# ubc-vision/StableKeypoints

Hardware: AMD Instinct MI355X
Metric: images/sec for token-optimization step (SD1.5, 512^2, K=10 kpts) (higher is better)
Workload: dtype f32 (fp32 MFMA / VALU throughout; flash attention of the >= 1024-key self-attention layers: 3xbf16 operand split, fp32 accumulate, error <= the fp32 kernel's)

## Files before the change

### stablekeypoints_amd/csrc/skp_flash_attn_s.hip

```cpp
#include "skp_attn_tiles.h"
#include <stdlib.h>

typedef __bf16 bf16x8 __attribute__((ext_vector_type(8)));

namespace {

template <int D>
struct FAS {
    static constexpr int G = (D + 15) / 16;
    static constexpr int KT = 64, NKT = 4;
    static constexpr int MAT_B = NKT * G * 2 * 1024;
    static constexpr int CHUNKS = MAT_B / 1024;
    static constexpr bool ONES = (D % 16) != 0;
};

__device__ __forceinline__ unsigned fas_cvt_pk(float lo, float hi) {
    unsigned r;
    asm("v_cvt_pk_bf16_f32 %0, %1, %2" : "=v"(r) : "v"(lo), "v"(hi));
    return r;
}
__device__ __forceinline__ void fas_split4(const f32x4 a, f32x4& mh, f32x4& hl) {
    unsigned h[2], m[2], l[2];
#pragma unroll
    for (int p = 0; p < 2; ++p) {
        const float x = a[2 * p], y = a[2 * p + 1];
        h[p] = fas_cvt_pk(x, y);
        const float rx = x - __builtin_bit_cast(float, h[p] << 16), ry = y - __builtin_bit_cast(float, h[p] & 0xffff0000u);
        m[p] = fas_cvt_pk(rx, ry);
        const float sx = rx - __builtin_bit_cast(float, m[p] << 16), sy = ry - __builtin_bit_cast(float, m[p] & 0xffff0000u);
        l[p] = fas_cvt_pk(sx, sy);
    }
    mh = f32x4{__builtin_bit_cast(float, m[0]), __builtin_bit_cast(float, h[0]), __builtin_bit_cast(float, m[1]), __builtin_bit_cast(float, h[1])};
    hl = f32x4{__builtin_bit_cast(float, h[0]), __builtin_bit_cast(float, l[0]), __builtin_bit_cast(float, h[1]), __builtin_bit_cast(float, l[1])};
}
__device__ __forceinline__ f32x4 fas_mfma(const f32x4& a, const f32x4& b, const f32x4& c) {
    return __builtin_amdgcn_mfma_f32_16x16x32_bf16(__builtin_bit_cast(bf16x8, a), __builtin_bit_cast(bf16x8, b), c, 0, 0, 0);
}

template <int D>
__global__ __launch_bounds__(256) void skp_fas_split_kernel(const float* __restrict__ k, const float* __restrict__ v, f32x4* __restrict__ Kt,
                                                           f32x4* __restrict__ Vt, int H, int Nk, int ntiles) {
    using F = FAS<D>;
    const int cell = blockIdx.x * 256 + threadIdx.x;
    const int lane = cell & 63, rest = cell >> 6;
    const int g = rest % F::G, kt = (rest / F::G) % F::NKT, tile = rest / (F::G * F::NKT);
    if (tile >= ntiles) return;
    const int h = blockIdx.y, bk = blockIdx.z, C = H * D;
    const int i16 = lane & 15, kq = lane >> 4;
    const float* kb = k + (size_t)bk * Nk * C + h * D;
    const float* vb = v + (size_t)bk * Nk * C + h * D;
    f32x4 a = {0.f, 0.f, 0.f, 0.f}, b = {0.f, 0.f, 0.f, 0.f};
    {
        const int t = tile * F::KT + 16 * kt + i16, c = 16 * g + 4 * kq;
        if (t < Nk && c < D) a = *(const f32x4*)(kb + (size_t)t * C + c);
    }
    {
        const int c = 16 * g + i16, t0 = tile * F::KT + 16 * kt + 4 * kq;
#pragma unroll
        for (int e = 0; e < 4; ++e)
            if (t0 + e < Nk) b[e] = c < D ? vb[(size_t)(t0 + e) * C + c] : (F::ONES && c == D ? 1.0f : 0.f);
    }
    f32x4 mh, hl;
    const size_t base = (((size_t)(bk * H + h) * ntiles + tile) * (F::MAT_B / 16)) + ((kt * F::G + g) * 2) * 64 + lane;
    fas_split4(a, mh, hl);
    Kt[base] = mh; Kt[base + 64] = hl;
    fas_split4(b, mh, hl);
    Vt[base] = mh; Vt[base + 64] = hl;
}

template <int D, int NQT>
__global__ __launch_bounds__(512, 2) void skp_fas_fwd_kernel(const float* __restrict__ q, const float* __restrict__ Kt, const float* __restrict__ Vt,
                                                            float* __restrict__ out, float* __restrict__ lse, int H, int N, int Nk,
                                                            int ntiles, int kvb, float scale) {
    using F = FAS<D>;
    extern __shared__ __attribute__((aligned(16))) unsigned char smem[];
    const int tid = threadIdx.x, lane = tid & 63, wave = __builtin_amdgcn_readfirstlane(tid >> 6);
    const int i16 = lane & 15, g = lane >> 4;
    const int b = blockIdx.z, h = blockIdx.y, C = H * D;
    const int nbase = blockIdx.x * (128 * NQT) + wave * (16 * NQT);
    const float sl2 = scale * SKP_LOG2E;
    const size_t img = (size_t)((kvb ? b : 0) * H + h) * ntiles * F::MAT_B;
    const i32x4 krs = skp_make_rsrc((const char*)Kt + img, (unsigned)((size_t)ntiles * F::MAT_B));
    const i32x4 vrs = skp_make_rsrc((const char*)Vt + img, (unsigned)((size_t)ntiles * F::MAT_B));

    f32x4 qmh[NQT][F::G], qhl[NQT][F::G];
    int nrow[NQT];
#pragma unroll
    for (int nt = 0; nt < NQT; ++nt) {
        const int n = nbase + 16 * nt + i16;
        nrow[nt] = n;
        const float* qrow = q + ((size_t)b * N + (n < N ? n : N - 1)) * C + h * D;
#pragma unroll
        for (int gg = 0; gg < F::G; ++gg) {
            const int c = 16 * gg + 4 * g;
            const f32x4 x = c < D ? *(const f32x4*)(qrow + c) * sl2 : f32x4{0.f, 0.f, 0.f, 0.f};
            fas_split4(x, qmh[nt][gg], qhl[nt][gg]);
        }
    }
    f32x4 o[F::G][NQT];
#pragma unroll
    for (int ct = 0; ct < F::G; ++ct)
#pragma unroll
        for (int nt = 0; nt < NQT; ++nt) o[ct][nt] = f32x4{0.f, 0.f, 0.f, 0.f};
    float mrun[NQT], lpart[NQT];
#pragma unroll
    for (int nt = 0; nt < NQT; ++nt) { mrun[nt] = -INFINITY; lpart[nt] = 0.f; }
    constexpr int LCT = D / 16, LG = (D % 16) / 4, LR = D % 4;

    auto stage = [&](int tile, int buf) {
        unsigned char* dst = smem + buf * 2 * F::MAT_B;
#pragma unroll
        for (int j = 0; j < (F::CHUNKS + 7) / 8; ++j) {
            const int p = j * 8 + wave;
            if (p < F::CHUNKS) {
                skp_buf_load_lds(krs, (skp_lds_ptr)(dst + p * 1024), 16, lane * 16, tile * F::MAT_B + p * 1024, 0, 0);
                skp_buf_load_lds(vrs, (skp_lds_ptr)(dst + F::MAT_B + p * 1024), 16, lane * 16, tile * F::MAT_B + p * 1024, 0, 0);
            }
        }
    };
    stage(0, 0);
    for (int tile = 0; tile < ntiles; ++tile) {
        const int cur = tile & 1;
        asm volatile("s_waitcnt vmcnt(0)" ::: "memory");
        __syncthreads();
        if (tile + 1 < ntiles) stage(tile + 1, cur ^ 1);
        const unsigned char* Ks = smem + cur * 2 * F::MAT_B + lane * 16;
        const unsigned char* Vs = Ks + F::MAT_B;
        const int kt0 = tile * F::KT;

        f32x4 s[F::NKT][NQT];
#pragma unroll
        for (int kt = 0; kt < F::NKT; ++kt) {
#pragma unroll
            for (int nt = 0; nt < NQT; ++nt) s[kt][nt] = f32x4{0.f, 0.f, 0.f, 0.f};
#pragma unroll
            for (int gg = 0; gg < F::G; ++gg) {
                const f32x4 kmh = *(const f32x4*)(Ks + ((kt * F::G + gg) * 2) * 1024);
                const f32x4 khl = *(const f32x4*)(Ks + ((kt * F::G + gg) * 2 + 1) * 1024);
#pragma unroll
                for (int nt = 0; nt < NQT; ++nt) s[kt][nt] = fas_mfma(kmh, qhl[nt][gg], s[kt][nt]);
#pragma unroll
                for (int nt = 0; nt < NQT; ++nt) s[kt][nt] = fas_mfma(khl, qmh[nt][gg], s[kt][nt]);
#pragma unroll
                for (int nt = 0; nt < NQT; ++nt) s[kt][nt] = fas_mfma(kmh, qmh[nt][gg], s[kt][nt]);
            }
        }
        if (kt0 + F::KT > Nk) {
            const int left = Nk - kt0;
#pragma unroll
            for (int kt = 0; kt < F::NKT; ++kt)
#pragma unroll
                for (int r = 0; r < 4; ++r)
                    if (16 * kt + 4 * g + r >= left) {
#pragma unroll
                        for (int nt = 0; nt < NQT; ++nt) s[kt][nt][r] = -INFINITY;
                    }
        }
#pragma unroll
        for (int nt = 0; nt < NQT; ++nt) {
            float tm = fmaxf(fmaxf(s[0][nt][0], s[0][nt][1]), fmaxf(s[0][nt][2], s[0][nt][3]));
#pragma unroll
            for (int kt = 1; kt < F::NKT; ++kt) tm = fmaxf(tm, fmaxf(fmaxf(s[kt][nt][0], s[kt][nt][1]), fmaxf(s[kt][nt][2], s[kt][nt][3])));
            tm = fmaxf(tm, __shfl_xor(tm, 16, 64));
            tm = fmaxf(tm, __shfl_xor(tm, 32, 64));
            const float mn = fmaxf(mrun[nt], tm);
            const float alpha = __builtin_amdgcn_exp2f(mrun[nt] - mn);
            mrun[nt] = mn;
            float rs = 0.f;
#pragma unroll
            for (int kt = 0; kt < F::NKT; ++kt)
#pragma unroll
                for (int r = 0; r < 4; ++r) {
                    s[kt][nt][r] = __builtin_amdgcn_exp2f(s[kt][nt][r] - mn);
                    if (!F::ONES) rs += s[kt][nt][r];
                }
            if (!F::ONES) lpart[nt] = lpart[nt] * alpha + rs;
#pragma unroll
            for (int ct = 0; ct < F::G; ++ct) o[ct][nt] *= alpha;
        }
#pragma unroll
        for (int kt = 0; kt < F::NKT; ++kt) {
            f32x4 pmh[NQT], phl[NQT];
#pragma unroll
            for (int nt = 0; nt < NQT; ++nt) fas_split4(s[kt][nt], pmh[nt], phl[nt]);
#pragma unroll
            for (int ct = 0; ct < F::G; ++ct) {
                const f32x4 vmh = *(const f32x4*)(Vs + ((kt * F::G + ct) * 2) * 1024);
                const f32x4 vhl = *(const f32x4*)(Vs + ((kt * F::G + ct) * 2 + 1) * 1024);
#pragma unroll
                for (int nt = 0; nt < NQT; ++nt) o[ct][nt] = fas_mfma(vmh, phl[nt], o[ct][nt]);
#pragma unroll
                for (int nt = 0; nt < NQT; ++nt) o[ct][nt] = fas_mfma(vhl, pmh[nt], o[ct][nt]);
#pragma unroll
                for (int nt = 0; nt < NQT; ++nt) o[ct][nt] = fas_mfma(vmh, pmh[nt], o[ct][nt]);
            }
        }
    }
#pragma unroll
    for (int nt = 0; nt < NQT; ++nt) {
        float l;
        if (F::ONES) l = __shfl(o[LCT][nt][LR], 16 * LG + i16, 64);
        else { l = lpart[nt]; l += __shfl_xor(l, 16, 64); l += __shfl_xor(l, 32, 64); }
        const float inv = 1.0f / l;
        const int n = nrow[nt];
        if (n < N) {
            float* orow = out + ((size_t)b * N + n) * C + h * D;
#pragma unroll
            for (int ct = 0; ct < F::G; ++ct) {
                const int c0 = 16 * ct + 4 * g;
                if (c0 < D) *(f32x4*)(orow + c0) = o[ct][nt] * inv;
            }
            if (g == 0) lse[((size_t)b * H + h) * N + n] = (mrun[nt] + __builtin_amdgcn_logf(l)) * SKP_LN2;
        }
    }
}

template <int D, int NB>
__global__ __launch_bounds__(256) void skp_fas_images_kernel(const float* __restrict__ x, f32x4* __restrict__ Xr, f32x4* __restrict__ Xt, int H,
                                                            int Nr, int ntiles, float mult) {
    using F = FAS<D>;
    constexpr int MAT16 = NB * F::G * 2 * 64;
    const int cell = blockIdx.x * 256 + threadIdx.x;
    const int lane = cell & 63, rest = cell >> 6;
    const int g = rest % F::G, nb = (rest / F::G) % NB, tile = rest / (F::G * NB);
    if (tile >= ntiles) return;
    const int h = blockIdx.y, b = blockIdx.z, C = H * D;
    const int i16 = lane & 15, kq = lane >> 4;
    const float* xb = x + (size_t)b * Nr * C + h * D;
    f32x4 a = {0.f, 0.f, 0.f, 0.f}, t4 = {0.f, 0.f, 0.f, 0.f};
    {
        const int r = tile * 16 * NB + 16 * nb + i16, c = 16 * g + 4 * kq;
        if (r < Nr && c < D) a = *(const f32x4*)(xb + (size_t)r * C + c) * mult;
    }
    {
        const int c = 16 * g + i16, r0 = tile * 16 * NB + 16 * nb + 4 * kq;
#pragma unroll
        for (int e = 0; e < 4; ++e)
            if (r0 + e < Nr && c < D) t4[e] = xb[(size_t)(r0 + e) * C + c] * mult;
    }
    f32x4 mh, hl;
    const size_t base = ((size_t)(b * H + h) * ntiles + tile) * MAT16 + ((nb * F::G + g) * 2) * 64 + lane;
    fas_split4(a, mh, hl);
    Xr[base] = mh; Xr[base + 64] = hl;
    fas_split4(t4, mh, hl);
    Xt[base] = mh; Xt[base + 64] = hl;
}

template <int D>
__global__ __launch_bounds__(512, 2) void skp_fas_bwd_dq_kernel(const float* __restrict__ q, const float* __restrict__ o, const float* __restrict__ dout,
                                                               const float* __restrict__ lse, const float* __restrict__ Kr,
                                                               const float* __restrict__ Vr, const float* __restrict__ Kt,
                                                               float* __restrict__ dq, float* __restrict__ Dn, int H, int N, int Nk,
                                                               int ntiles, float scale, int ldg) {
    using F = FAS<D>;
    constexpr int NQT = 2;
    extern __shared__ __attribute__((aligned(16))) unsigned char smem[];
    const int tid = threadIdx.x, lane = tid & 63, wave = __builtin_amdgcn_readfirstlane(tid >> 6);
    const int i16 = lane & 15, g = lane >> 4;
    const int b = blockIdx.z, h = blockIdx.y, C = H * D;
    const int nbase = blockIdx.x * 256 + wave * (16 * NQT);
    const float sl2 = scale * SKP_LOG2E;
    const size_t img = (size_t)(b * H + h) * ntiles * F::MAT_B;
    const i32x4 krs = skp_make_rsrc((const char*)Kr + img, (unsigned)((size_t)ntiles * F::MAT_B));
    const i32x4 vrs = skp_make_rsrc((const char*)Vr + img, (unsigned)((size_t)ntiles * F::MAT_B));
    const i32x4 trs = skp_make_rsrc((const char*)Kt + img, (unsigned)((size_t)ntiles * F::MAT_B));

    f32x4 qmh[NQT][F::G], qhl[NQT][F::G], gmh[NQT][F::G], ghl[NQT][F::G];
    float lse2[NQT], dsum[NQT];
    int nrow[NQT];
#pragma unroll
    for (int nt = 0; nt < NQT; ++nt) {
        const int n = nbase + 16 * nt + i16;
        nrow[nt] = n;
        const size_t ro = ((size_t)b * N + (n < N ? n : N - 1)) * C + h * D;
        float dpart = 0.f;
#pragma unroll
        for (int gg = 0; gg < F::G; ++gg) {
            const int c = 16 * gg + 4 * g;
            f32x4 x = {0.f, 0.f, 0.f, 0.f}, gv = {0.f, 0.f, 0.f, 0.f}, ov = {0.f, 0.f, 0.f, 0.f};
            if (c < D) { x = *(const f32x4*)(q + ro + c) * sl2; gv = *(const f32x4*)(dout + ro + c); ov = *(const f32x4*)(o + ro + c); }
            fas_split4(x, qmh[nt][gg], qhl[nt][gg]);
            fas_split4(gv, gmh[nt][gg], ghl[nt][gg]);
            dpart += gv[0] * ov[0] + gv[1] * ov[1] + gv[2] * ov[2] + gv[3] * ov[3];
        }
        dpart += __shfl_xor(dpart, 16, 64);
        dpart += __shfl_xor(dpart, 32, 64);
        dsum[nt] = dpart;
        lse2[nt] = lse[((size_t)b * H + h) * N + (n < N ? n : N - 1)] * SKP_LOG2E;
        if (g == 0 && n < N) Dn[((size_t)b * H + h) * N + n] = dpart;
    }
    f32x4 acc[F::G][NQT];
#pragma unroll
    for (int ct = 0; ct < F::G; ++ct)
#pragma unroll
        for (int nt = 0; nt < NQT; ++nt) acc[ct][nt] = f32x4{0.f, 0.f, 0.f, 0.f};

    auto stage = [&](int tile, int buf) {
        unsigned char* dst = smem + buf * 3 * F::MAT_B;
#pragma unroll
        for (int j = 0; j < (F::CHUNKS + 7) / 8; ++j) {
            const int p = j * 8 + wave;
            if (p < F::CHUNKS) {
                skp_buf_load_lds(krs, (skp_lds_ptr)(dst + p * 1024), 16, lane * 16, tile * F::MAT_B + p * 1024, 0, 0);
                skp_buf_load_lds(vrs, (skp_lds_ptr)(dst + F::MAT_B + p * 1024), 16, lane * 16, tile * F::MAT_B + p * 1024, 0, 0);
                skp_buf_load_lds(trs, (skp_lds_ptr)(dst + 2 * F::MAT_B + p * 1024), 16, lane * 16, tile * F::MAT_B + p * 1024, 0, 0);
            }
        }
    };
    stage(0, 0);
    for (int tile = 0; tile < ntiles; ++tile) {
        const int cur = tile & 1;
        asm volatile("s_waitcnt vmcnt(0)" ::: "memory");
        __syncthreads();
        if (tile + 1 < ntiles) stage(tile + 1, cur ^ 1);
        const unsigned char* Ks = smem + cur * 3 * F::MAT_B + lane * 16;
        const unsigned char* Vs = Ks + F::MAT_B;
        const unsigned char* Ts = Ks + 2 * F::MAT_B;
        const int left = Nk - tile * F::KT;
#pragma unroll
        for (int kt = 0; kt < F::NKT; ++kt) {
            f32x4 s[NQT], dp[NQT];
#pragma unroll
            for (int nt = 0; nt < NQT; ++nt) { s[nt] = f32x4{0.f, 0.f, 0.f, 0.f}; dp[nt] = f32x4{0.f, 0.f, 0.f, 0.f}; }
#pragma unroll
            for (int gg = 0; gg < F::G; ++gg) {
                const f32x4 kmh = *(const f32x4*)(Ks + ((kt * F::G + gg) * 2) * 1024);
                const f32x4 khl = *(const f32x4*)(Ks + ((kt * F::G + gg) * 2 + 1) * 1024);
                const f32x4 vmh = *(const f32x4*)(Vs + ((kt * F::G + gg) * 2) * 1024);
                const f32x4 vhl = *(const f32x4*)(Vs + ((kt * F::G + gg) * 2 + 1) * 1024);
#pragma unroll
                for (int nt = 0; nt < NQT; ++nt) { s[nt] = fas_mfma(kmh, qhl[nt][gg], s[nt]); dp[nt] = fas_mfma(vmh, ghl[nt][gg], dp[nt]); }
#pragma unroll
                for (int nt = 0; nt < NQT; ++nt) { s[nt] = fas_mfma(khl, qmh[nt][gg], s[nt]); dp[nt] = fas_mfma(vhl, gmh[nt][gg], dp[nt]); }
#pragma unroll
                for (int nt = 0; nt < NQT; ++nt) { s[nt] = fas_mfma(kmh, qmh[nt][gg], s[nt]); dp[nt] = fas_mfma(vmh, gmh[nt][gg], dp[nt]); }
            }
            f32x4 dmh[NQT], dhl[NQT];
#pragma unroll
            for (int nt = 0; nt < NQT; ++nt) {
                f32x4 ds;
#pragma unroll
                for (int r = 0; r < 4; ++r) {
                    const float p = (16 * kt + 4 * g + r < left) ? __builtin_amdgcn_exp2f(s[nt][r] - lse2[nt]) : 0.f;
                    ds[r] = p * (dp[nt][r] - dsum[nt]);
                }
                fas_split4(ds, dmh[nt], dhl[nt]);
            }
#pragma unroll
            for (int ct = 0; ct < F::G; ++ct) {
                const f32x4 tmh = *(const f32x4*)(Ts + ((kt * F::G + ct) * 2) * 1024);
                const f32x4 thl = *(const f32x4*)(Ts + ((kt * F::G + ct) * 2 + 1) * 1024);
#pragma unroll
                for (int nt = 0; nt < NQT; ++nt) acc[ct][nt] = fas_mfma(tmh, dhl[nt], acc[ct][nt]);
#pragma unroll
                for (int nt = 0; nt < NQT; ++nt) acc[ct][nt] = fas_mfma(thl, dmh[nt], acc[ct][nt]);
#pragma unroll
                for (int nt = 0; nt < NQT; ++nt) acc[ct][nt] = fas_mfma(tmh, dmh[nt], acc[ct][nt]);
            }
        }
    }
#pragma unroll
    for (int nt = 0; nt < NQT; ++nt) {
        const int n = nrow[nt];
        if (n < N) {
            float* drow = dq + ((size_t)b * N + n) * ldg + h * D;
#pragma unroll
            for (int ct = 0; ct < F::G; ++ct) {
                const int c0 = 16 * ct + 4 * g;
                if (c0 < D) *(f32x4*)(drow + c0) = acc[ct][nt] * scale;
            }
        }
    }
}

template <int D>
__global__ __launch_bounds__(512, 2) void skp_fas_bwd_dkv_kernel(const float* __restrict__ k, const float* __restrict__ v, const float* __restrict__ lse,
                                                                const float* __restrict__ Dn, const float* __restrict__ Qr,
                                                                const float* __restrict__ Gr, const float* __restrict__ Qt,
                                                                const float* __restrict__ Gt, float* __restrict__ dk, float* __restrict__ dv,
                                                                int H, int N, int Nk, int nqtiles, float scale, int ldg) {
    using F = FAS<D>;
    constexpr int NKB = 2, NB = 2;
    constexpr int QMAT = NB * F::G * 2 * 1024;
    constexpr int QCH = QMAT / 1024;
    extern __shared__ __attribute__((aligned(16))) unsigned char smem[];
    const int tid = threadIdx.x, lane = tid & 63, wave = __builtin_amdgcn_readfirstlane(tid >> 6);
    const int i16 = lane & 15, g = lane >> 4;
    const int b = blockIdx.z, h = blockIdx.y, C = H * D;
    const int tbase = blockIdx.x * 256 + wave * (16 * NKB);
    const size_t img = (size_t)(b * H + h) * nqtiles * QMAT;
    const i32x4 qrs = skp_make_rsrc((const char*)Qr + img, (unsigned)((size_t)nqtiles * QMAT));
    const i32x4 grs = skp_make_rsrc((const char*)Gr + img, (unsigned)((size_t)nqtiles * QMAT));
    const i32x4 qts = skp_make_rsrc((const char*)Qt + img, (unsigned)((size_t)nqtiles * QMAT));
    const i32x4 gts = skp_make_rsrc((const char*)Gt + img, (unsigned)((size_t)nqtiles * QMAT));
    const float* lrow = lse + ((size_t)b * H + h) * N;
    const float* drow = Dn + ((size_t)b * H + h) * N;

    f32x4 kmh[NKB][F::G], khl[NKB][F::G], vmh[NKB][F::G], vhl[NKB][F::G];
    int trow[NKB];
#pragma unroll
    for (int kb = 0; kb < NKB; ++kb) {
        const int t = tbase + 16 * kb + i16;
        trow[kb] = t;
        const size_t ro = ((size_t)b * Nk + (t < Nk ? t : Nk - 1)) * C + h * D;
#pragma unroll
        for (int gg = 0; gg < F::G; ++gg) {
            const int c = 16 * gg + 4 * g;
            f32x4 x = {0.f, 0.f, 0.f, 0.f}, y = {0.f, 0.f, 0.f, 0.f};
            if (c < D && t < Nk) { x = *(const f32x4*)(k + ro + c); y = *(const f32x4*)(v + ro + c); }
            fas_split4(x, kmh[kb][gg], khl[kb][gg]);
            fas_split4(y, vmh[kb][gg], vhl[kb][gg]);
        }
    }
    f32x4 ak[F::G][NKB], av[F::G][NKB];
#pragma unroll
    for (int ct = 0; ct < F::G; ++ct)
#pragma unroll
        for (int kb = 0; kb < NKB; ++kb) { ak[ct][kb] = f32x4{0.f, 0.f, 0.f, 0.f}; av[ct][kb] = f32x4{0.f, 0.f, 0.f, 0.f}; }

    auto stage = [&](int tile, int buf) {
        unsigned char* dst = smem + buf * 4 * QMAT;
#pragma unroll
        for (int j = 0; j < (QCH + 7) / 8; ++j) {
            const int p = j * 8 + wave;
            if (p < QCH) {
                skp_buf_load_lds(qrs, (skp_lds_ptr)(dst + p * 1024), 16, lane * 16, tile * QMAT + p * 1024, 0, 0);
                skp_buf_load_lds(grs, (skp_lds_ptr)(dst + QMAT + p * 1024), 16, lane * 16, tile * QMAT + p * 1024, 0, 0);
                skp_buf_load_lds(qts, (skp_lds_ptr)(dst + 2 * QMAT + p * 1024), 16, lane * 16, tile * QMAT + p * 1024, 0, 0);
                skp_buf_load_lds(gts, (skp_lds_ptr)(dst + 3 * QMAT + p * 1024), 16, lane * 16, tile * QMAT + p * 1024, 0, 0);
            }
        }
    };
    stage(0, 0);
    for (int tile = 0; tile < nqtiles; ++tile) {
        const int cur = tile & 1;
        f32x4 l2[NB], dn[NB];
#pragma unroll
        for (int nb = 0; nb < NB; ++nb) {
            const int n0 = tile * 16 * NB + 16 * nb + 4 * g;
#pragma unroll
            for (int r = 0; r < 4; ++r) {
                const int n = n0 + r;
                l2[nb][r] = n < N ? lrow[n] * SKP_LOG2E : INFINITY;
                dn[nb][r] = n < N ? drow[n] : 0.f;
            }
        }
        asm volatile("s_waitcnt vmcnt(0)" ::: "memory");
        __syncthreads();
        if (tile + 1 < nqtiles) stage(tile + 1, cur ^ 1);
        const unsigned char* Qs = smem + cur * 4 * QMAT + lane * 16;
        const unsigned char* Gs = Qs + QMAT;
        const unsigned char* Qts = Qs + 2 * QMAT;
        const unsigned char* Gts = Qs + 3 * QMAT;
#pragma unroll
        for (int nb = 0; nb < NB; ++nb) {
            f32x4 s[NKB], dp[NKB];
#pragma unroll
            for (int kb = 0; kb < NKB; ++kb) { s[kb] = f32x4{0.f, 0.f, 0.f, 0.f}; dp[kb] = f32x4{0.f, 0.f, 0.f, 0.f}; }
#pragma unroll
            for (int gg = 0; gg < F::G; ++gg) {
                const f32x4 qm = *(const f32x4*)(Qs + ((nb * F::G + gg) * 2) * 1024);
                const f32x4 qh = *(const f32x4*)(Qs + ((nb * F::G + gg) * 2 + 1) * 1024);
                const f32x4 gm = *(const f32x4*)(Gs + ((nb * F::G + gg) * 2) * 1024);
                const f32x4 gh = *(const f32x4*)(Gs + ((nb * F::G + gg) * 2 + 1) * 1024);
#pragma unroll
                for (int kb = 0; kb < NKB; ++kb) { s[kb] = fas_mfma(qm, khl[kb][gg], s[kb]); dp[kb] = fas_mfma(gm, vhl[kb][gg], dp[kb]); }
#pragma unroll
                for (int kb = 0; kb < NKB; ++kb) { s[kb] = fas_mfma(qh, kmh[kb][gg], s[kb]); dp[kb] = fas_mfma(gh, vmh[kb][gg], dp[kb]); }
#pragma unroll
                for (int kb = 0; kb < NKB; ++kb) { s[kb] = fas_mfma(qm, kmh[kb][gg], s[kb]); dp[kb] = fas_mfma(gm, vmh[kb][gg], dp[kb]); }
            }
            f32x4 pmh[NKB], phl[NKB], dmh[NKB], dhl[NKB];
#pragma unroll
            for (int kb = 0; kb < NKB; ++kb) {
                f32x4 p, ds;
#pragma unroll
                for (int r = 0; r < 4; ++r) {
                    p[r] = __builtin_amdgcn_exp2f(s[kb][r] - l2[nb][r]);
                    ds[r] = p[r] * (dp[kb][r] - dn[nb][r]);
                }
                fas_split4(p, pmh[kb], phl[kb]);
                fas_split4(ds, dmh[kb], dhl[kb]);
            }
#pragma unroll
            for (int ct = 0; ct < F::G; ++ct) {
                const f32x4 tm = *(const f32x4*)(Qts + ((nb * F::G + ct) * 2) * 1024);
                const f32x4 th = *(const f32x4*)(Qts + ((nb * F::G + ct) * 2 + 1) * 1024);
                const f32x4 um = *(const f32x4*)(Gts + ((nb * F::G + ct) * 2) * 1024);
                const f32x4 uh = *(const f32x4*)(Gts + ((nb * F::G + ct) * 2 + 1) * 1024);
#pragma unroll
                for (int kb = 0; kb < NKB; ++kb) { ak[ct][kb] = fas_mfma(tm, dhl[kb], ak[ct][kb]); av[ct][kb] = fas_mfma(um, phl[kb], av[ct][kb]); }
#pragma unroll
                for (int kb = 0; kb < NKB; ++kb) { ak[ct][kb] = fas_mfma(th, dmh[kb], ak[ct][kb]); av[ct][kb] = fas_mfma(uh, pmh[kb], av[ct][kb]); }
#pragma unroll
                for (int kb = 0; kb < NKB; ++kb) { ak[ct][kb] = fas_mfma(tm, dmh[kb], ak[ct][kb]); av[ct][kb] = fas_mfma(um, pmh[kb], av[ct][kb]); }
            }
        }
    }
#pragma unroll
    for (int kb = 0; kb < NKB; ++kb) {
        const int t = trow[kb];
        if (t < Nk) {
            float* krow = dk + ((size_t)b * Nk + t) * ldg + h * D;
            float* vrow = dv + ((size_t)b * Nk + t) * ldg + h * D;
#pragma unroll
            for (int ct = 0; ct < F::G; ++ct) {
                const int c0 = 16 * ct + 4 * g;
                if (c0 < D) {
                    *(f32x4*)(krow + c0) = ak[ct][kb] * SKP_LN2;
                    *(f32x4*)(vrow + c0) = av[ct][kb];
                }
            }
        }
    }
}

template <int D>
static int fas_bwd_run(const float* q, const float* k, const float* v, const float* o, const float* dout, const float* lse, float* dq,
                       float* dk, float* dv, void* workspace, int B, int H, int N, float scale, int ldg, hipStream_t st) {
    using F = FAS<D>;
    const int ntiles = (N + F::KT - 1) / F::KT, nqtiles = (N + 31) / 32;
    const size_t kimg = (size_t)B * H * ntiles * F::MAT_B;
    const size_t qimg = (size_t)B * H * nqtiles * (F::MAT_B / 2);
    char* w = (char*)workspace;
    f32x4 *Kr = (f32x4*)w, *Kt = (f32x4*)(w + kimg), *Vr = (f32x4*)(w + 2 * kimg), *Vt = (f32x4*)(w + 3 * kimg);
    f32x4 *Qr = (f32x4*)(w + 4 * kimg), *Qt = (f32x4*)(w + 4 * kimg + qimg), *Gr = (f32x4*)(w + 4 * kimg + 2 * qimg),
          *Gt = (f32x4*)(w + 4 * kimg + 3 * qimg);
    float* Dn = (float*)(w + 4 * kimg + 4 * qimg);
    const int kcells = ntiles * F::NKT * F::G * 64, qcells = nqtiles * 2 * F::G * 64;
    hipLaunchKernelGGL((skp_fas_images_kernel<D, 4>), dim3((kcells + 255) / 256, H, B), dim3(256), 0, st, k, Kr, Kt, H, N, ntiles, 1.0f);
    hipLaunchKernelGGL((skp_fas_images_kernel<D, 4>), dim3((kcells + 255) / 256, H, B), dim3(256), 0, st, v, Vr, Vt, H, N, ntiles, 1.0f);
    hipLaunchKernelGGL((skp_fas_images_kernel<D, 2>), dim3((qcells + 255) / 256, H, B), dim3(256), 0, st, q, Qr, Qt, H, N, nqtiles, scale * SKP_LOG2E);
    hipLaunchKernelGGL((skp_fas_images_kernel<D, 2>), dim3((qcells + 255) / 256, H, B), dim3(256), 0, st, dout, Gr, Gt, H, N, nqtiles, 1.0f);
    const size_t lds_q = (size_t)6 * F::MAT_B, lds_k = (size_t)8 * (F::MAT_B / 2);
    static bool attr_set = false;
    if (!attr_set) {
        hipError_t e = hipFuncSetAttribute((const void*)skp_fas_bwd_dq_kernel<D>, hipFuncAttributeMaxDynamicSharedMemorySize, (int)lds_q);
        if (e != hipSuccess) return (int)e;
        e = hipFuncSetAttribute((const void*)skp_fas_bwd_dkv_kernel<D>, hipFuncAttributeMaxDynamicSharedMemorySize, (int)lds_k);
        if (e != hipSuccess) return (int)e;
        attr_set = true;
    }
    hipLaunchKernelGGL(skp_fas_bwd_dq_kernel<D>, dim3((N + 255) / 256, H, B), dim3(512), lds_q, st, q, o, dout, lse, (const float*)Kr,
                       (const float*)Vr, (const float*)Kt, dq, Dn, H, N, N, ntiles, scale, ldg);
    hipLaunchKernelGGL(skp_fas_bwd_dkv_kernel<D>, dim3((N + 255) / 256, H, B), dim3(512), lds_k, st, k, v, lse, (const float*)Dn,
                       (const float*)Qr, (const float*)Gr, (const float*)Qt, (const float*)Gt, dk, dv, H, N, N, nqtiles, scale, ldg);
    return skp_launch_status();
}

template <int D, int NQT>
static int fas_run(const float* q, const float* k, const float* v, float* out, float* lse, void* workspace, int B, int Bk, int H, int N,
                   int Nk, float scale, hipStream_t st) {
    using F = FAS<D>;
    const int ntiles = (Nk + F::KT - 1) / F::KT;
    const size_t img = (size_t)Bk * H * ntiles * F::MAT_B;
    f32x4* Kt = (f32x4*)workspace;
    f32x4* Vt = (f32x4*)((char*)workspace + img);
    const int cells = ntiles * F::NKT * F::G * 64;
    hipLaunchKernelGGL(skp_fas_split_kernel<D>, dim3((cells + 255) / 256, H, Bk), dim3(256), 0, st, k, v, Kt, Vt, H, Nk, ntiles);
    const size_t lds = (size_t)4 * F::MAT_B;
    static bool attr_set = false;
    if (!attr_set) {
        hipError_t e = hipFuncSetAttribute((const void*)skp_fas_fwd_kernel<D, NQT>, hipFuncAttributeMaxDynamicSharedMemorySize, (int)lds);
        if (e != hipSuccess) return (int)e;
        attr_set = true;
    }
    hipLaunchKernelGGL((skp_fas_fwd_kernel<D, NQT>), dim3((N + 128 * NQT - 1) / (128 * NQT), H, B), dim3(512), lds, st, q, (const float*)Kt, (const float*)Vt, out, lse,
                       H, N, Nk, ntiles, Bk == B && B > 1 ? 1 : 0, scale);
    return skp_launch_status();
}

}

extern "C" int skp_flash_attn_fwd_split_ok(int B, int Bk, int H, int N, int Nk, int d) {
    if (B <= 0 || H <= 0 || N <= 0 || Nk <= 0 || (Bk != 1 && Bk != B)) return 0;
    if (d != 40 && d != 80) return 0;
    const long long ntiles = (Nk + 63) / 64, mat = 4ll * ((d + 15) / 16) * 2 * 1024;
    return ntiles * mat < 0x7fffffffll ? 1 : 0;
}

extern "C" int64_t skp_flash_attn_fwd_split_workspace(int B, int Bk, int H, int N, int Nk, int d) {
    if (!skp_flash_attn_fwd_split_ok(B, Bk, H, N, Nk, d)) return 0;
    const int64_t ntiles = (Nk + 63) / 64, mat = (int64_t)4 * ((d + 15) / 16) * 2 * 1024;
    return 2 * (int64_t)Bk * H * ntiles * mat;
}

extern "C" int skp_flash_attn_fwd_split_f32(const float* q, const float* k, const float* v, float* out, float* lse, void* workspace,
                                            int B, int Bk, int H, int N, int Nk, int d, float scale, void* stream) {
    if (!q || !k || !v || !out || !lse || !workspace) return SKP_E_BADARG;
    if (B <= 0 || H <= 0 || N <= 0 || Nk <= 0 || (Bk != 1 && Bk != B)) return SKP_E_BADARG;
    if (!skp_flash_attn_fwd_split_ok(B, Bk, H, N, Nk, d)) return SKP_E_RANGE;
    hipStream_t st = (hipStream_t)stream;
    const bool small = (long)((N + 255) / 256) * H * B < 256;
    if (d == 40) return small ? fas_run<40, 1>(q, k, v, out, lse, workspace, B, Bk, H, N, Nk, scale, st)
                              : fas_run<40, 2>(q, k, v, out, lse, workspace, B, Bk, H, N, Nk, scale, st);
    return small ? fas_run<80, 1>(q, k, v, out, lse, workspace, B, Bk, H, N, Nk, scale, st)
                 : fas_run<80, 2>(q, k, v, out, lse, workspace, B, Bk, H, N, Nk, scale, st);
}

extern "C" int skp_flash_attn_bwd_split_ok(int B, int Bk, int H, int N, int Nk, int d) {
    if (B <= 0 || H <= 0 || N <= 0 || Bk != B || Nk != N || d != 40) return 0;
    const long long ntiles = (N + 63) / 64, mat = 4ll * ((d + 15) / 16) * 2 * 1024;
    return ntiles * mat < 0x7fffffffll ? 1 : 0;
}
extern "C" int64_t skp_flash_attn_bwd_split_workspace(int B, int Bk, int H, int N, int Nk, int d) {
    if (!skp_flash_attn_bwd_split_ok(B, Bk, H, N, Nk, d)) return 0;
    const int64_t mat = (int64_t)4 * ((d + 15) / 16) * 2 * 1024;
    return 4 * (int64_t)B * H * ((N + 63) / 64) * mat + 4 * (int64_t)B * H * ((N + 31) / 32) * (mat / 2) + (int64_t)B * H * N * 4;
}
extern "C" int skp_flash_attn_bwd_split_f32(const float* q, const float* k, const float* v, const float* out, const float* dout,
                                            const float* lse, float* dq, float* dk, float* dv, void* workspace, int B, int Bk, int H,
                                            int N, int Nk, int d, float scale, void* stream) {
    if (!q || !k || !v || !out || !dout || !lse || !dq || !dk || !dv || !workspace) return SKP_E_BADARG;
    if (!skp_flash_attn_bwd_split_ok(B, Bk, H, N, Nk, d)) return SKP_E_RANGE;
    return fas_bwd_run<40>(q, k, v, out, dout, lse, dq, dk, dv, workspace, B, H, N, scale, H * d, (hipStream_t)stream);
}
extern "C" int skp_flash_attn_bwd_split_ld_f32(const float* q, const float* k, const float* v, const float* out, const float* dout,
                                               const float* lse, float* dq, float* dk, float* dv, void* workspace, int B, int Bk, int H,
                                               int N, int Nk, int d, float scale, int ldg, void* stream) {
    if (!q || !k || !v || !out || !dout || !lse || !dq || !dk || !dv || !workspace) return SKP_E_BADARG;
    if (ldg < H * d || (ldg & 3)) return SKP_E_BADARG;
    if (!skp_flash_attn_bwd_split_ok(B, Bk, H, N, Nk, d)) return SKP_E_RANGE;
    return fas_bwd_run<40>(q, k, v, out, dout, lse, dq, dk, dv, workspace, B, H, N, scale, ldg, (hipStream_t)stream);
}
```

Before: 54.43.

## Software-pipeline flash-attention backward kernels and merge split-image launches

The dq kernel is software-pipelined across key sub-tiles: scores for the next sub-tile are computed while the previous one's dS accumulation runs, with sched_group_barrier hints pinning how MFMA and VALU work interleave. The dkv kernel moves to a three-slot ring for Q/G row images and a separate double buffer for transposed images, prefetches lse/D rows one tile ahead, and interleaves the two query blocks' score, softmax and accumulate phases. The four bf16-split image launches are merged into two, and the V transpose image that is never read is no longer written. The compiler's bf16 conversion is also used in place of inline asm, and lane indices are recomputed at the epilogue to free registers. The costs are more LDS per dkv block and higher register pressure from the pipelined buffers, which could reduce occupancy.

```diff
diff --git a/stablekeypoints_amd/csrc/skp_flash_attn_s.hip b/stablekeypoints_amd/csrc/skp_flash_attn_s.hip
--- a/stablekeypoints_amd/csrc/skp_flash_attn_s.hip
+++ b/stablekeypoints_amd/csrc/skp_flash_attn_s.hip
@@ -2,6 +2,7 @@
 #include <stdlib.h>
 
 typedef __bf16 bf16x8 __attribute__((ext_vector_type(8)));
+typedef __bf16 bf16x2 __attribute__((ext_vector_type(2)));
 
 namespace {
 
@@ -19,22 +20,50 @@
     asm("v_cvt_pk_bf16_f32 %0, %1, %2" : "=v"(r) : "v"(lo), "v"(hi));
     return r;
 }
+__device__ __forceinline__ unsigned fas_cvt_pk_vis(float lo, float hi) {
+    return __builtin_bit_cast(unsigned, __builtin_convertvector(f32x2{lo, hi}, bf16x2));
+}
+template <bool VIS = false>
 __device__ __forceinline__ void fas_split4(const f32x4 a, f32x4& mh, f32x4& hl) {
     unsigned h[2], m[2], l[2];
 #pragma unroll
     for (int p = 0; p < 2; ++p) {
         const float x = a[2 * p], y = a[2 * p + 1];
-        h[p] = fas_cvt_pk(x, y);
+        h[p] = VIS ? fas_cvt_pk_vis(x, y) : fas_cvt_pk(x, y);
         const float rx = x - __builtin_bit_cast(float, h[p] << 16), ry = y - __builtin_bit_cast(float, h[p] & 0xffff0000u);
-        m[p] = fas_cvt_pk(rx, ry);
+        m[p] = VIS ? fas_cvt_pk_vis(rx, ry) : fas_cvt_pk(rx, ry);
         const float sx = rx - __builtin_bit_cast(float, m[p] << 16), sy = ry - __builtin_bit_cast(float, m[p] & 0xffff0000u);
-        l[p] = fas_cvt_pk(sx, sy);
+        l[p] = VIS ? fas_cvt_pk_vis(sx, sy) : fas_cvt_pk(sx, sy);
     }
     mh = f32x4{__builtin_bit_cast(float, m[0]), __builtin_bit_cast(float, h[0]), __builtin_bit_cast(float, m[1]), __builtin_bit_cast(float, h[1])};
     hl = f32x4{__builtin_bit_cast(float, h[0]), __builtin_bit_cast(float, l[0]), __builtin_bit_cast(float, h[1]), __builtin_bit_cast(float, l[1])};
 }
+__device__ __forceinline__ int fas_lane_again() {
+    int l = __builtin_amdgcn_mbcnt_hi(~0u, __builtin_amdgcn_mbcnt_lo(~0u, 0u));
+    asm volatile("" : "+v"(l));
+    return l;
+}
 __device__ __forceinline__ f32x4 fas_mfma(const f32x4& a, const f32x4& b, const f32x4& c) {
     return __builtin_amdgcn_mfma_f32_16x16x32_bf16(__builtin_bit_cast(bf16x8, a), __builtin_bit_cast(bf16x8, b), c, 0, 0, 0);
+}
+
+template <int NG, int ND, int NM, int NV>
+__device__ __forceinline__ void fas_pin() {
+    __builtin_amdgcn_sched_group_barrier(0x100, ND, 0);
+#pragma unroll
+    for (int i = 0; i < NG; ++i) {
+        __builtin_amdgcn_sched_group_barrier(0x100, ND, 0);
+#pragma unroll
+        for (int j = 0; j < NM; ++j) {
+            __builtin_amdgcn_sched_group_barrier(0x008, 1, 0);
+            if (NV > 0) __builtin_amdgcn_sched_group_barrier(0x002, NV, 0);
+        }
+    }
+}
+template <int NG, int ND, int NM, int NV>
+__device__ __forceinline__ void fas_region_end() {
+    fas_pin<NG, ND, NM, NV>();
+    __builtin_amdgcn_sched_barrier(0);
 }
 
 template <int D>
@@ -215,16 +244,23 @@
     }
 }
 
-template <int D, int NB>
-__global__ __launch_bounds__(256) void skp_fas_images_kernel(const float* __restrict__ x, f32x4* __restrict__ Xr, f32x4* __restrict__ Xt, int H,
-                                                            int Nr, int ntiles, float mult) {
+template <int D, int NB, bool T1>
+__global__ __launch_bounds__(256) void skp_fas_images_kernel(const float* __restrict__ x0, const float* __restrict__ x1, f32x4* __restrict__ Xr0,
+                                                            f32x4* __restrict__ Xt0, f32x4* __restrict__ Xr1, f32x4* __restrict__ Xt1, int H,
+                                                            int Nr, int ntiles, float mult0, float mult1) {
     using F = FAS<D>;
     constexpr int MAT16 = NB * F::G * 2 * 64;
-    const int cell = blockIdx.x * 256 + threadIdx.x;
+    const int nblk = gridDim.x >> 1;
+    const bool second = (int)blockIdx.x >= nblk;
+    const int cell = (blockIdx.x - (second ? nblk : 0)) * 256 + threadIdx.x;
     const int lane = cell & 63, rest = cell >> 6;
     const int g = rest % F::G, nb = (rest / F::G) % NB, tile = rest / (F::G * NB);
     if (tile >= ntiles) return;
     const int h = blockIdx.y, b = blockIdx.z, C = H * D;
+    const float* x = second ? x1 : x0;
+    f32x4* Xr = second ? Xr1 : Xr0;
+    f32x4* Xt = second ? Xt1 : Xt0;
+    const float mult = second ? mult1 : mult0;
     const int i16 = lane & 15, kq = lane >> 4;
     const float* xb = x + (size_t)b * Nr * C + h * D;
     f32x4 a = {0.f, 0.f, 0.f, 0.f}, t4 = {0.f, 0.f, 0.f, 0.f};
@@ -232,16 +268,17 @@
         const int r = tile * 16 * NB + 16 * nb + i16, c = 16 * g + 4 * kq;
         if (r < Nr && c < D) a = *(const f32x4*)(xb + (size_t)r * C + c) * mult;
     }
-    {
-        const int c = 16 * g + i16, r0 = tile * 16 * NB + 16 * nb + 4 * kq;
-#pragma unroll
-        for (int e = 0; e < 4; ++e)
-            if (r0 + e < Nr && c < D) t4[e] = xb[(size_t)(r0 + e) * C + c] * mult;
-    }
     f32x4 mh, hl;
     const size_t base = ((size_t)(b * H + h) * ntiles + tile) * MAT16 + ((nb * F::G + g) * 2) * 64 + lane;
     fas_split4(a, mh, hl);
     Xr[base] = mh; Xr[base + 64] = hl;
+    if (!T1 && second) return;
+    {
+        const int c = 16 * g + i16, r0 = tile * 16 * NB + 16 * nb + 4 * kq;
+#pragma unroll
+        for (int e = 0; e < 4; ++e)
+            if (r0 + e < Nr && c < D) t4[e] = xb[(size_t)(r0 + e) * C + c] * mult;
+    }
     fas_split4(t4, mh, hl);
     Xt[base] = mh; Xt[base + 64] = hl;
 }
@@ -267,11 +304,9 @@
 
     f32x4 qmh[NQT][F::G], qhl[NQT][F::G], gmh[NQT][F::G], ghl[NQT][F::G];
     float lse2[NQT], dsum[NQT];
-    int nrow[NQT];
 #pragma unroll
     for (int nt = 0; nt < NQT; ++nt) {
         const int n = nbase + 16 * nt + i16;
-        nrow[nt] = n;
         const size_t ro = ((size_t)b * N + (n < N ? n : N - 1)) * C + h * D;
         float dpart = 0.f;
 #pragma unroll
@@ -279,8 +314,8 @@
             const int c = 16 * gg + 4 * g;
             f32x4 x = {0.f, 0.f, 0.f, 0.f}, gv = {0.f, 0.f, 0.f, 0.f}, ov = {0.f, 0.f, 0.f, 0.f};
             if (c < D) { x = *(const f32x4*)(q + ro + c) * sl2; gv = *(const f32x4*)(dout + ro + c); ov = *(const f32x4*)(o + ro + c); }
-            fas_split4(x, qmh[nt][gg], qhl[nt][gg]);
-            fas_split4(gv, gmh[nt][gg], ghl[nt][gg]);
+            fas_split4<true>(x, qmh[nt][gg], qhl[nt][gg]);
+            fas_split4<true>(gv, gmh[nt][gg], ghl[nt][gg]);
             dpart += gv[0] * ov[0] + gv[1] * ov[1] + gv[2] * ov[2] + gv[3] * ov[3];
         }
         dpart += __shfl_xor(dpart, 16, 64);
@@ -317,9 +352,7 @@
         const unsigned char* Vs = Ks + F::MAT_B;
         const unsigned char* Ts = Ks + 2 * F::MAT_B;
         const int left = Nk - tile * F::KT;
-#pragma unroll
-        for (int kt = 0; kt < F::NKT; ++kt) {
-            f32x4 s[NQT], dp[NQT];
+        auto scores = [&](int kt, f32x4 (&s)[NQT], f32x4 (&dp)[NQT]) __attribute__((always_inline)) {
 #pragma unroll
             for (int nt = 0; nt < NQT; ++nt) { s[nt] = f32x4{0.f, 0.f, 0.f, 0.f}; dp[nt] = f32x4{0.f, 0.f, 0.f, 0.f}; }
 #pragma unroll
@@ -335,17 +368,20 @@
 #pragma unroll
                 for (int nt = 0; nt < NQT; ++nt) { s[nt] = fas_mfma(kmh, qmh[nt][gg], s[nt]); dp[nt] = fas_mfma(vmh, gmh[nt][gg], dp[nt]); }
             }
-            f32x4 dmh[NQT], dhl[NQT];
+        };
+        auto dsplit = [&](int kt, const f32x4 (&s)[NQT], const f32x4 (&dp)[NQT], f32x4 (&dmh)[NQT], f32x4 (&dhl)[NQT]) __attribute__((always_inline)) {
 #pragma unroll
             for (int nt = 0; nt < NQT; ++nt) {
                 f32x4 ds;
 #pragma unroll
                 for (int r = 0; r < 4; ++r) {
-                    const float p = (16 * kt + 4 * g + r < left) ? __builtin_amdgcn_exp2f(s[nt][r] - lse2[nt]) : 0.f;
+                    const float p = (4 * g < left - 16 * kt - r) ? __builtin_amdgcn_exp2f(s[nt][r] - lse2[nt]) : 0.f;
                     ds[r] = p * (dp[nt][r] - dsum[nt]);
                 }
-                fas_split4(ds, dmh[nt], dhl[nt]);
-            }
+                fas_split4<true>(ds, dmh[nt], dhl[nt]);
+            }
+        };
+        auto accum = [&](int kt, const f32x4 (&dmh)[NQT], const f32x4 (&dhl)[NQT]) __attribute__((always_inline)) {
 #pragma unroll
             for (int ct = 0; ct < F::G; ++ct) {
                 const f32x4 tmh = *(const f32x4*)(Ts + ((kt * F::G + ct) * 2) * 1024);
@@ -357,16 +393,30 @@
 #pragma unroll
                 for (int nt = 0; nt < NQT; ++nt) acc[ct][nt] = fas_mfma(tmh, dmh[nt], acc[ct][nt]);
             }
-        }
-    }
+        };
+        f32x4 s[2][NQT], dp[2][NQT], dmh[2][NQT], dhl[2][NQT];
+        scores(0, s[0], dp[0]);
+        fas_region_end<F::G, 4, 6 * NQT, 0>();
+#pragma unroll
+        for (int kt = 0; kt < F::NKT; ++kt) {
+            if (kt + 1 < F::NKT) scores(kt + 1, s[(kt + 1) & 1], dp[(kt + 1) & 1]);
+            if (kt > 0) accum(kt - 1, dmh[(kt - 1) & 1], dhl[(kt - 1) & 1]);
+            dsplit(kt, s[kt & 1], dp[kt & 1], dmh[kt & 1], dhl[kt & 1]);
+            if (kt + 1 < F::NKT) fas_pin<F::G, 4, 6 * NQT, 2>();
+            if (kt > 0) fas_pin<F::G, 2, 3 * NQT, 2>();
+            __builtin_amdgcn_sched_barrier(0);
+        }
+        accum(F::NKT - 1, dmh[(F::NKT - 1) & 1], dhl[(F::NKT - 1) & 1]);
+    }
+    const int elane = fas_lane_again(), ei16 = elane & 15, eg = elane >> 4;
 #pragma unroll
     for (int nt = 0; nt < NQT; ++nt) {
-        const int n = nrow[nt];
+        const int n = nbase + 16 * nt + ei16;
         if (n < N) {
             float* drow = dq + ((size_t)b * N + n) * ldg + h * D;
 #pragma unroll
             for (int ct = 0; ct < F::G; ++ct) {
-                const int c0 = 16 * ct + 4 * g;
+                const int c0 = 16 * ct + 4 * eg;
                 if (c0 < D) *(f32x4*)(drow + c0) = acc[ct][nt] * scale;
             }
         }
@@ -397,19 +447,17 @@
     const float* drow = Dn + ((size_t)b * H + h) * N;
 
     f32x4 kmh[NKB][F::G], khl[NKB][F::G], vmh[NKB][F::G], vhl[NKB][F::G];
-    int trow[NKB];
 #pragma unroll
     for (int kb = 0; kb < NKB; ++kb) {
         const int t = tbase + 16 * kb + i16;
-        trow[kb] = t;
         const size_t ro = ((size_t)b * Nk + (t < Nk ? t : Nk - 1)) * C + h * D;
 #pragma unroll
         for (int gg = 0; gg < F::G; ++gg) {
             const int c = 16 * gg + 4 * g;
             f32x4 x = {0.f, 0.f, 0.f, 0.f}, y = {0.f, 0.f, 0.f, 0.f};
             if (c < D && t < Nk) { x = *(const f32x4*)(k + ro + c); y = *(const f32x4*)(v + ro + c); }
-            fas_split4(x, kmh[kb][gg], khl[kb][gg]);
-            fas_split4(y, vmh[kb][gg], vhl[kb][gg]);
+            fas_split4<true>(x, kmh[kb][gg], khl[kb][gg]);
+            fas_split4<true>(y, vmh[kb][gg], vhl[kb][gg]);
         }
     }
     f32x4 ak[F::G][NKB], av[F::G][NKB];
@@ -418,94 +466,142 @@
 #pragma unroll
         for (int kb = 0; kb < NKB; ++kb) { ak[ct][kb] = f32x4{0.f, 0.f, 0.f, 0.f}; av[ct][kb] = f32x4{0.f, 0.f, 0.f, 0.f}; }
 
-    auto stage = [&](int tile, int buf) {
-        unsigned char* dst = smem + buf * 4 * QMAT;
+    auto stage_r = [&](int tile, int slot) __attribute__((always_inline)) {
+        unsigned char* dst = smem + slot * 2 * QMAT;
 #pragma unroll
         for (int j = 0; j < (QCH + 7) / 8; ++j) {
             const int p = j * 8 + wave;
             if (p < QCH) {
                 skp_buf_load_lds(qrs, (skp_lds_ptr)(dst + p * 1024), 16, lane * 16, tile * QMAT + p * 1024, 0, 0);
                 skp_buf_load_lds(grs, (skp_lds_ptr)(dst + QMAT + p * 1024), 16, lane * 16, tile * QMAT + p * 1024, 0, 0);
-                skp_buf_load_lds(qts, (skp_lds_ptr)(dst + 2 * QMAT + p * 1024), 16, lane * 16, tile * QMAT + p * 1024, 0, 0);
-                skp_buf_load_lds(gts, (skp_lds_ptr)(dst + 3 * QMAT + p * 1024), 16, lane * 16, tile * QMAT + p * 1024, 0, 0);
-            }
-        }
-    };
-    stage(0, 0);
+            }
+        }
+    };
+    auto stage_t = [&](int tile, int slot) __attribute__((always_inline)) {
+        unsigned char* dst = smem + 6 * QMAT + slot * 2 * QMAT;
+#pragma unroll
+        for (int j = 0; j < (QCH + 7) / 8; ++j) {
+            const int p = j * 8 + wave;
+            if (p < QCH) {
+                skp_buf_load_lds(qts, (skp_lds_ptr)(dst + p * 1024), 16, lane * 16, tile * QMAT + p * 1024, 0, 0);
+                skp_buf_load_lds(gts, (skp_lds_ptr)(dst + QMAT + p * 1024), 16, lane * 16, tile * QMAT + p * 1024, 0, 0);
+            }
+        }
+    };
+    auto load_ld = [&](int tile, f32x4 (&lr)[NB], f32x4 (&dr)[NB]) __attribute__((always_inline)) {
+#pragma unroll
+        for (int nb = 0; nb < NB; ++nb)
+#pragma unroll
+            for (int r = 0; r < 4; ++r) {
+                const int n = tile * 16 * NB + 16 * nb + 4 * g + r, nc = n < N ? n : N - 1;
+                lr[nb][r] = lrow[nc];
+                dr[nb][r] = drow[nc];
+            }
+    };
+    auto scores = [&](const unsigned char* Rs, int nb, f32x4 (&s)[NKB], f32x4 (&dp)[NKB]) __attribute__((always_inline)) {
+        const unsigned char* Gs = Rs + QMAT;
+#pragma unroll
+        for (int kb = 0; kb < NKB; ++kb) { s[kb] = f32x4{0.f, 0.f, 0.f, 0.f}; dp[kb] = f32x4{0.f, 0.f, 0.f, 0.f}; }
+#pragma unroll
+        for (int gg = 0; gg < F::G; ++gg) {
+            const f32x4 qm = *(const f32x4*)(Rs + ((nb * F::G + gg) * 2) * 1024);
+            const f32x4 qh = *(const f32x4*)(Rs + ((nb * F::G + gg) * 2 + 1) * 1024);
+            const f32x4 gm = *(const f32x4*)(Gs + ((nb * F::G + gg) * 2) * 1024);
+            const f32x4 gh = *(const f32x4*)(Gs + ((nb * F::G + gg) * 2 + 1) * 1024);
+#pragma unroll
+            for (int kb = 0; kb < NKB; ++kb) { s[kb] = fas_mfma(qm, khl[kb][gg], s[kb]); dp[kb] = fas_mfma(gm, vhl[kb][gg], dp[kb]); }
+#pragma unroll
+            for (int kb = 0; kb < NKB; ++kb) { s[kb] = fas_mfma(qh, kmh[kb][gg], s[kb]); dp[kb] = fas_mfma(gh, vmh[kb][gg], dp[kb]); }
+#pragma unroll
+            for (int kb = 0; kb < NKB; ++kb) { s[kb] = fas_mfma(qm, kmh[kb][gg], s[kb]); dp[kb] = fas_mfma(gm, vmh[kb][gg], dp[kb]); }
+        }
+    };
+    auto psplit = [&](const f32x4 (&s)[NKB], const f32x4& l2, f32x4 (&p)[NKB], f32x4 (&pmh)[NKB], f32x4 (&phl)[NKB]) __attribute__((always_inline)) {
+#pragma unroll
+        for (int kb = 0; kb < NKB; ++kb) {
+#pragma unroll
+            for (int r = 0; r < 4; ++r) p[kb][r] = __builtin_amdgcn_exp2f(s[kb][r] - l2[r]);
+            fas_split4<true>(p[kb], pmh[kb], phl[kb]);
+        }
+    };
+    auto dsplit = [&](const f32x4 (&p)[NKB], const f32x4 (&dp)[NKB], const f32x4& dn, f32x4 (&dmh)[NKB], f32x4 (&dhl)[NKB]) __attribute__((always_inline)) {
+#pragma unroll
+        for (int kb = 0; kb < NKB; ++kb) {
+            f32x4 ds;
+#pragma unroll
+            for (int r = 0; r < 4; ++r) ds[r] = p[kb][r] * (dp[kb][r] - dn[r]);
+            fas_split4<true>(ds, dmh[kb], dhl[kb]);
+        }
+    };
+    auto accum = [&](const unsigned char* Ts, int nb, const f32x4 (&pmh)[NKB], const f32x4 (&phl)[NKB], const f32x4 (&dmh)[NKB],
+                     const f32x4 (&dhl)[NKB]) __attribute__((always_inline)) {
+        const unsigned char* Us = Ts + QMAT;
+#pragma unroll
+        for (int ct = 0; ct < F::G; ++ct) {
+            const f32x4 tm = *(const f32x4*)(Ts + ((nb * F::G + ct) * 2) * 1024);
+            const f32x4 th = *(const f32x4*)(Ts + ((nb * F::G + ct) * 2 + 1) * 1024);
+            const f32x4 um = *(const f32x4*)(Us + ((nb * F::G + ct) * 2) * 1024);
+            const f32x4 uh = *(const f32x4*)(Us + ((nb * F::G + ct) * 2 + 1) * 1024);
+#pragma unroll
+            for (int kb = 0; kb < NKB; ++kb) { ak[ct][kb] = fas_mfma(tm, dhl[kb], ak[ct][kb]); av[ct][kb] = fas_mfma(um, phl[kb], av[ct][kb]); }
+#pragma unroll
+            for (int kb = 0; kb < NKB; ++kb) { ak[ct][kb] = fas_mfma(th, dmh[kb], ak[ct][kb]); av[ct][kb] = fas_mfma(uh, pmh[kb], av[ct][kb]); }
+#pragma unroll
+            for (int kb = 0; kb < NKB; ++kb) { ak[ct][kb] = fas_mfma(tm, dmh[kb], ak[ct][kb]); av[ct][kb] = fas_mfma(um, pmh[kb], av[ct][kb]); }
+        }
+    };
+    static_assert(NB == 2, "the loop body below is written out for two query blocks per tile");
+    stage_r(0, 0);
+    stage_t(0, 0);
+    if (nqtiles > 1) stage_r(1, 1);
+    f32x4 lrn[NB], drn[NB];
+    load_ld(0, lrn, drn);
+    asm volatile("s_waitcnt vmcnt(0)" ::: "memory");
+    __syncthreads();
+    f32x4 s0[NKB], dp0[NKB], s1[NKB], dp1[NKB];
+    scores(smem + lane * 16, 0, s0, dp0);
+    int ra = 0;
     for (int tile = 0; tile < nqtiles; ++tile) {
-        const int cur = tile & 1;
-        f32x4 l2[NB], dn[NB];
-#pragma unroll
-        for (int nb = 0; nb < NB; ++nb) {
-            const int n0 = tile * 16 * NB + 16 * nb + 4 * g;
-#pragma unroll
-            for (int r = 0; r < 4; ++r) {
-                const int n = n0 + r;
-                l2[nb][r] = n < N ? lrow[n] * SKP_LOG2E : INFINITY;
-                dn[nb][r] = n < N ? drow[n] : 0.f;
-            }
-        }
+        const int rb = ra == 2 ? 0 : ra + 1, rc = rb == 2 ? 0 : rb + 1;
         asm volatile("s_waitcnt vmcnt(0)" ::: "memory");
         __syncthreads();
-        if (tile + 1 < nqtiles) stage(tile + 1, cur ^ 1);
-        const unsigned char* Qs = smem + cur * 4 * QMAT + lane * 16;
-        const unsigned char* Gs = Qs + QMAT;
-        const unsigned char* Qts = Qs + 2 * QMAT;
-        const unsigned char* Gts = Qs + 3 * QMAT;
-#pragma unroll
-        for (int nb = 0; nb < NB; ++nb) {
-            f32x4 s[NKB], dp[NKB];
-#pragma unroll
-            for (int kb = 0; kb < NKB; ++kb) { s[kb] = f32x4{0.f, 0.f, 0.f, 0.f}; dp[kb] = f32x4{0.f, 0.f, 0.f, 0.f}; }
-#pragma unroll
-            for (int gg = 0; gg < F::G; ++gg) {
-                const f32x4 qm = *(const f32x4*)(Qs + ((nb * F::G + gg) * 2) * 1024);
-                const f32x4 qh = *(const f32x4*)(Qs + ((nb * F::G + gg) * 2 + 1) * 1024);
-                const f32x4 gm = *(const f32x4*)(Gs + ((nb * F::G + gg) * 2) * 1024);
-                const f32x4 gh = *(const f32x4*)(Gs + ((nb * F::G + gg) * 2 + 1) * 1024);
-#pragma unroll
-                for (int kb = 0; kb < NKB; ++kb) { s[kb] = fas_mfma(qm, khl[kb][gg], s[kb]); dp[kb] = fas_mfma(gm, vhl[kb][gg], dp[kb]); }
-#pragma unroll
-                for (int kb = 0; kb < NKB; ++kb) { s[kb] = fas_mfma(qh, kmh[kb][gg], s[kb]); dp[kb] = fas_mfma(gh, vmh[kb][gg], dp[kb]); }
-#pragma unroll
-                for (int kb = 0; kb < NKB; ++kb) { s[kb] = fas_mfma(qm, kmh[kb][gg], s[kb]); dp[kb] = fas_mfma(gm, vmh[kb][gg], dp[kb]); }
-            }
-            f32x4 pmh[NKB], phl[NKB], dmh[NKB], dhl[NKB];
-#pragma unroll
-            for (int kb = 0; kb < NKB; ++kb) {
-                f32x4 p, ds;
-#pragma unroll
-                for (int r = 0; r < 4; ++r) {
-                    p[r] = __builtin_amdgcn_exp2f(s[kb][r] - l2[nb][r]);
-                    ds[r] = p[r] * (dp[kb][r] - dn[nb][r]);
-                }
-                fas_split4(p, pmh[kb], phl[kb]);
-                fas_split4(ds, dmh[kb], dhl[kb]);
-            }
-#pragma unroll
-            for (int ct = 0; ct < F::G; ++ct) {
-                const f32x4 tm = *(const f32x4*)(Qts + ((nb * F::G + ct) * 2) * 1024);
-                const f32x4 th = *(const f32x4*)(Qts + ((nb * F::G + ct) * 2 + 1) * 1024);
-                const f32x4 um = *(const f32x4*)(Gts + ((nb * F::G + ct) * 2) * 1024);
-                const f32x4 uh = *(const f32x4*)(Gts + ((nb * F::G + ct) * 2 + 1) * 1024);
-#pragma unroll
-                for (int kb = 0; kb < NKB; ++kb) { ak[ct][kb] = fas_mfma(tm, dhl[kb], ak[ct][kb]); av[ct][kb] = fas_mfma(um, phl[kb], av[ct][kb]); }
-#pragma unroll
-                for (int kb = 0; kb < NKB; ++kb) { ak[ct][kb] = fas_mfma(th, dmh[kb], ak[ct][kb]); av[ct][kb] = fas_mfma(uh, pmh[kb], av[ct][kb]); }
-#pragma unroll
-                for (int kb = 0; kb < NKB; ++kb) { ak[ct][kb] = fas_mfma(tm, dmh[kb], ak[ct][kb]); av[ct][kb] = fas_mfma(um, pmh[kb], av[ct][kb]); }
-            }
-        }
-    }
+        f32x4 l2[NB], dn[NB];
+#pragma unroll
+        for (int nb = 0; nb < NB; ++nb)
+#pragma unroll
+            for (int r = 0; r < 4; ++r) {
+                const bool in = tile * 16 * NB + 16 * nb + 4 * g + r < N;
+                l2[nb][r] = in ? lrn[nb][r] * SKP_LOG2E : INFINITY;
+                dn[nb][r] = in ? drn[nb][r] : 0.f;
+            }
+        if (tile + 2 < nqtiles) stage_r(tile + 2, rc);
+        if (tile + 1 < nqtiles) stage_t(tile + 1, (tile + 1) & 1);
+        load_ld(tile + 1, lrn, drn);
+        const unsigned char* Ra = smem + ra * 2 * QMAT + lane * 16;
+        const unsigned char* Rb = smem + rb * 2 * QMAT + lane * 16;
+        const unsigned char* Ts = smem + 6 * QMAT + (tile & 1) * 2 * QMAT + lane * 16;
+        f32x4 p[NKB], pmh[NKB], phl[NKB], dmh[NKB], dhl[NKB];
+        scores(Ra, 1, s1, dp1);
+        psplit(s0, l2[0], p, pmh, phl);
+        dsplit(p, dp0, dn[0], dmh, dhl);
+        accum(Ts, 0, pmh, phl, dmh, dhl);
+        f32x4 p1[NKB], pmh1[NKB], phl1[NKB], dmh1[NKB], dhl1[NKB];
+        psplit(s1, l2[1], p1, pmh1, phl1);
+        scores(Rb, 0, s0, dp0);
+        dsplit(p1, dp1, dn[1], dmh1, dhl1);
+        accum(Ts, 1, pmh1, phl1, dmh1, dhl1);
+        ra = rb;
+    }
+    const int elane = fas_lane_again(), ei16 = elane & 15, eg = elane >> 4;
 #pragma unroll
     for (int kb = 0; kb < NKB; ++kb) {
-        const int t = trow[kb];
+        const int t = tbase + 16 * kb + ei16;
         if (t < Nk) {
             float* krow = dk + ((size_t)b * Nk + t) * ldg + h * D;
             float* vrow = dv + ((size_t)b * Nk + t) * ldg + h * D;
 #pragma unroll
             for (int ct = 0; ct < F::G; ++ct) {
-                const int c0 = 16 * ct + 4 * g;
+                const int c0 = 16 * ct + 4 * eg;
                 if (c0 < D) {
                     *(f32x4*)(krow + c0) = ak[ct][kb] * SKP_LN2;
                     *(f32x4*)(vrow + c0) = av[ct][kb];
@@ -523,16 +619,16 @@
     const size_t kimg = (size_t)B * H * ntiles * F::MAT_B;
     const size_t qimg = (size_t)B * H * nqtiles * (F::MAT_B / 2);
     char* w = (char*)workspace;
-    f32x4 *Kr = (f32x4*)w, *Kt = (f32x4*)(w + kimg), *Vr = (f32x4*)(w + 2 * kimg), *Vt = (f32x4*)(w + 3 * kimg);
+    f32x4 *Kr = (f32x4*)w, *Kt = (f32x4*)(w + kimg), *Vr = (f32x4*)(w + 2 * kimg);
     f32x4 *Qr = (f32x4*)(w + 4 * kimg), *Qt = (f32x4*)(w + 4 * kimg + qimg), *Gr = (f32x4*)(w + 4 * kimg + 2 * qimg),
           *Gt = (f32x4*)(w + 4 * kimg + 3 * qimg);
     float* Dn = (float*)(w + 4 * kimg + 4 * qimg);
     const int kcells = ntiles * F::NKT * F::G * 64, qcells = nqtiles * 2 * F::G * 64;
-    hipLaunchKernelGGL((skp_fas_images_kernel<D, 4>), dim3((kcells + 255) / 256, H, B), dim3(256), 0, st, k, Kr, Kt, H, N, ntiles, 1.0f);
-    hipLaunchKernelGGL((skp_fas_images_kernel<D, 4>), dim3((kcells + 255) / 256, H, B), dim3(256), 0, st, v, Vr, Vt, H, N, ntiles, 1.0f);
-    hipLaunchKernelGGL((skp_fas_images_kernel<D, 2>), dim3((qcells + 255) / 256, H, B), dim3(256), 0, st, q, Qr, Qt, H, N, nqtiles, scale * SKP_LOG2E);
-    hipLaunchKernelGGL((skp_fas_images_kernel<D, 2>), dim3((qcells + 255) / 256, H, B), dim3(256), 0, st, dout, Gr, Gt, H, N, nqtiles, 1.0f);
-    const size_t lds_q = (size_t)6 * F::MAT_B, lds_k = (size_t)8 * (F::MAT_B / 2);
+    hipLaunchKernelGGL((skp_fas_images_kernel<D, 4, false>), dim3(2 * ((kcells + 255) / 256), H, B), dim3(256), 0, st, k, v, Kr, Kt, Vr, (f32x4*)nullptr,
+                       H, N, ntiles, 1.0f, 1.0f);
+    hipLaunchKernelGGL((skp_fas_images_kernel<D, 2, true>), dim3(2 * ((qcells + 255) / 256), H, B), dim3(256), 0, st, q, dout, Qr, Qt, Gr, Gt, H, N,
+                       nqtiles, scale * SKP_LOG2E, 1.0f);
+    const size_t lds_q = (size_t)6 * F::MAT_B, lds_k = (size_t)10 * (F::MAT_B / 2);
     static bool attr_set = false;
     if (!attr_set) {
         hipError_t e = hipFuncSetAttribute((const void*)skp_fas_bwd_dq_kernel<D>, hipFuncAttributeMaxDynamicSharedMemorySize, (int)lds_q);
```

After: 54.42, median of 2. No clear change (-0.0%).
